# ReubenBond/DistributedRateLimiting.Redis

Hardware: AMD Instinct MI355X
Metric: acquire decisions/sec (node) at 100M keys, 1/2/4/8 GPU; % HBM roofline (higher is better)
Workload: dtype f64; 1 GPU; TokenBucket uniform keys, 2^26-request batches (config B); keys_total=100000000, keys_per_gpu=100000000, batch_per_gpu=67108864, period_ticks=10000000, partitioning=one GPU owns every key

## Files before the change

distributedratelimiting.redis_amd/csrc/tbe_engine.hip:

```cpp
#include <hip/hip_runtime.h>

#include <algorithm>
#include <cmath>
#include <cstdarg>
#include <cstdio>
#include <cstdlib>
#include <cstring>
#include <new>
#include <string>
#include <thread>
#include <tuple>
#include <type_traits>
#include <vector>

#include "../../include/tbe.h"
#include "tbe_device.hpp"
#include "tbe_codec.hpp"
#include "tbe_numfmt.hpp"
#include "tbe_retry.hpp"

#pragma clang fp contract(off)

using namespace tbe;

// ... 96 lines not shown
        const uint32_t k = (uint32_t)v;
        if (k == key) return (nb + (uint32_t)(v >> 32)) << r_bits;
        if (k == kHotEmpty) return key;
        h = (h + 1) & (kHotSlots - 1);
    }
}

template <int N, typename KeyT>
__device__ __forceinline__ void hot_sortkeys(const KeyT (&kv)[N], const uint64_t *slots, uint32_t nb,
                                             int r_bits, uint32_t (&sk)[N]) {
    constexpr int G = N < 4 ? N : 4;
    static_assert(N % G == 0, "groups of G requests");
#pragma unroll
    for (int g = 0; g < N; g += G) {
        uint64_t v1[G], v2[G];
#pragma unroll
        for (int u = 0; u < G; ++u) {
            v1[u] = slots[hot_h1((uint32_t)kv[g + u])];
            v2[u] = slots[hot_h2((uint32_t)kv[g + u])];
        }
#pragma unroll
        for (int u = 0; u < G; ++u) {
            const uint32_t key = (uint32_t)kv[g + u];
            const bool in1 = (uint32_t)v1[u] == key;
            const uint64_t v = in1 ? v1[u] : v2[u];
            sk[g + u] = (in1 || (uint32_t)v2[u] == key) ? (nb + (uint32_t)(v >> 32)) << r_bits : key;
        }
    }
    return;
    uint64_t v[N];
#pragma unroll
    for (int it = 0; it < N; ++it) v[it] = slots[hot_hash((uint32_t)kv[it])];
#pragma unroll
    for (int it = 0; it < N; ++it) {
        const uint32_t key = (uint32_t)kv[it];
        const uint32_t k = (uint32_t)v[it];
        if (k == key) sk[it] = (nb + (uint32_t)(v[it] >> 32)) << r_bits;
        else if (k == kHotEmpty) sk[it] = key;
        else sk[it] = hot_sortkey(key, slots, nb, r_bits);
    }
}

constexpr int kHBlock = 512;
constexpr int kHItems = kTile / kHBlock;
#ifndef TBE_HIST_AHEAD
#define TBE_HIST_AHEAD 1
#endif
#ifndef TBE_HIST_WAVES
#define TBE_HIST_WAVES 8
#endif
#ifndef TBE_HIST_HOT_WAVES
#define TBE_HIST_HOT_WAVES 6
#endif
template <typename KeyT, bool HOT = false>
__global__ __launch_bounds__(kHBlock, HOT ? TBE_HIST_HOT_WAVES : TBE_HIST_WAVES) void k_hist(const KeyT *__restrict__ keys, uint64_t n,
                                                  int shift, uint32_t tiles_per_blk,
                                                  uint32_t ntiles, uint32_t *__restrict__ tileprefix,
                                                  uint32_t *__restrict__ blocksum, uint64_t n_keys,
                                                  uint32_t *__restrict__ err, int validate,
                                                  uint64_t kmask, const HotSet *__restrict__ hot = nullptr,
                                                  uint32_t nb = 0, int r_bits = 0,
                                                  uint32_t *__restrict__ bcount = nullptr,
                                                  int lowbits = 0, uint32_t nbt = 0,
                                                  uint8_t *__restrict__ dig_out = nullptr) {
    __shared__ uint32_t h8[kDigits * 8];
    __shared__ uint32_t tile_lo[2];
    static_assert(kHBlock == 2 * kDigits && kDigits * 8 == 4 * kHBlock, "two threads per digit; 4 counters each");
    __shared__ uint64_t hs[HOT ? kHotLds : 1];
    const int tid = threadIdx.x;
    const bool dig = tid < kDigits;
    const bool any_hot = HOT && hot_load<kHBlock>(hot, hs);
    const uint32_t t0 = blockIdx.x * tiles_per_blk;
    const uint32_t t1 = min(t0 + tiles_per_blk, ntiles);
    uint32_t run = 0;
    uint32_t acc = 0, acc_lo = 0;
    bool bad = false;
    KeyT kn[kHItems];
#if TBE_HIST_AHEAD >= 2
    KeyT kn2[kHItems];
#endif
    auto load_into = [&](KeyT (&dst)[kHItems], uint32_t t) {
#pragma unroll
        for (int it = 0; it < kHItems; ++it) {
            const uint64_t i = (uint64_t)t * kTile + it * kHBlock + tid;
            dst[it] = (t < t1 && i < n) ? LD_P(keys + i) : (KeyT)0;
        }
    };
    load_into(kn, t0);
#if TBE_HIST_AHEAD >= 2
    load_into(kn2, t0 + 1);
#endif
    for (uint32_t t = t0; t < t1; ++t) {
        KeyT kv[kHItems];
#pragma unroll
        for (int it = 0; it < kHItems; ++it) kv[it] = kn[it];
#if TBE_HIST_AHEAD >= 2
#pragma unroll
        for (int it = 0; it < kHItems; ++it) kn[it] = kn2[it];
        load_into(kn2, t + 2);
#else
        load_into(kn, t + 1);
#endif
#pragma unroll
        for (int u = 0; u < 4; ++u) h8[u * kHBlock + tid] = 0;
        __syncthreads();
        const uint64_t base = (uint64_t)t * kTile;
        const uint64_t last = min<uint64_t>(base + kTile, n) - 1;
        uint32_t skv[kHItems];
        if (HOT && any_hot) {
            hot_sortkeys<kHItems>(kv, hot_table(hot, hs), nb, r_bits, skv);
        } else {
#pragma unroll
            for (int it = 0; it < kHItems; ++it) skv[it] = (uint32_t)((uint64_t)kv[it] & kmask);
        }
#pragma unroll
        for (int it = 0; it < kHItems; ++it) {
            const uint64_t i = base + it * kHBlock + tid;
            const bool valid = i < n;
            const uint32_t sk = skv[it];
            const uint32_t d = (sk >> shift) & (kDigits - 1);
            const uint64_t vmask = __ballot(valid);
            const uint32_t d0 = __shfl(d, vmask ? __ffsll((long long)vmask) - 1 : 0, 64);
            if (__all(!valid || d == d0)) {
                if (vmask && (vmask & lanemask_lt()) == 0 && valid) atomicAdd(&h8[d0 * 8], (uint32_t)__popcll(vmask));
            } else {
                if (valid) atomicAdd(&h8[d * 8 + (tid & 7)], 1u);
            }
            if (dig_out && valid) dig_out[i] = (uint8_t)d;
            if (valid) {
                bad |= validate && ((uint64_t)kv[it] >= n_keys);
                if (bcount && (i == base || i == last)) {
                    tile_lo[i == last] = lowbits ? (sk >> r_bits) & ((1u << lowbits) - 1u) : 0u;
                    if (i == base && i == last) tile_lo[0] = tile_lo[1];
                }
            }
        }
        __syncthreads();
        uint32_t c = 0;
        if (dig) {
#pragma unroll
            for (int u = 0; u < 8; ++u) c += h8[tid * 8 + ((u + tid) & 7)];
            tileprefix[(uint64_t)t * kDigits + tid] = run;
            run += c;
        }
        if (bcount) {
            const uint32_t lo0 = tile_lo[0], lo1 = tile_lo[1];
            if (lo0 == lo1) {
                if (dig) {
                    if (lo0 != acc_lo) {
                        const uint32_t bk = ((uint32_t)tid << lowbits) | acc_lo;
                        if (acc && bk < nbt) atomicAdd(&bcount[bk], acc);
                        acc = 0;
                        acc_lo = lo0;
                    }
                    acc += c;
                }
            } else if (lo1 - lo0 < 8) {
                __syncthreads();
#pragma unroll
                for (int u = 0; u < 4; ++u) h8[u * kHBlock + tid] = 0;
                __syncthreads();
#pragma unroll
                for (int it = 0; it < kHItems; ++it) {
                    const uint64_t i = base + it * kHBlock + tid;
                    const uint32_t bk = skv[it] >> r_bits;
                    if (i < n) atomicAdd(&h8[((bk & ((1u << lowbits) - 1u)) - lo0) * kDigits + ((bk >> lowbits) & (kDigits - 1))], 1u);
                }
                __syncthreads();
                if (dig) {
                    for (uint32_t u = 0; u <= lo1 - lo0; ++u) {
                        const uint32_t cnt = h8[u * kDigits + tid];
                        const uint32_t bk = ((uint32_t)tid << lowbits) | (lo0 + u);
                        if (cnt && bk < nbt) atomicAdd(&bcount[bk], cnt);
                    }
                }
            } else {
#pragma unroll
                for (int it = 0; it < kHItems; ++it) {
                    const uint64_t i = base + it * kHBlock + tid;
                    const uint32_t bk = skv[it] >> r_bits;
                    if (i < n && bk < nbt) atomicAdd(&bcount[bk], 1u);
                }
            }
        }
        __syncthreads();
    }
    if (bcount && dig) {
        const uint32_t bk = ((uint32_t)tid << lowbits) | acc_lo;
        if (acc && bk < nbt) atomicAdd(&bcount[bk], acc);
    }
    if (dig) blocksum[(uint64_t)blockIdx.x * kDigits + tid] = run;
    if (__any(bad) && (tid & 63) == 0) atomicOr(err, 1u);
}

__global__ __launch_bounds__(kHBlock, TBE_HIST_WAVES) void k_hist_dig(
    const uint8_t *__restrict__ dig, uint64_t n, uint32_t tiles_per_blk, uint32_t ntiles,
    uint32_t *__restrict__ tileprefix, uint32_t *__restrict__ blocksum,
    const uint32_t *__restrict__ dtot0, uint32_t *__restrict__ bcount, uint32_t nbt) {
    __shared__ uint32_t h8[kDigits * 8];
    __shared__ uint32_t dstart[kDigits + 1];
    __shared__ uint32_t wsum[kHBlock / 64];
    __shared__ uint32_t tlo[kHBlock];
    static_assert(kHBlock == 2 * kDigits && kDigits * 8 == 4 * kHBlock, "two threads per digit; 4 counters each");
    static_assert(kHItems % 8 == 0, "8-byte loads");
    constexpr int kW = kHItems / 8;
    const int tid = threadIdx.x;
    const bool own = tid < kDigits;
    {
        uint32_t all;
        const uint32_t pre = block_excl_scan<kHBlock>(own ? dtot0[tid] : 0u, wsum, &all);
        if (own) dstart[tid] = pre;
        if (tid == 0) dstart[kDigits] = 0xFFFFFFFFu;
    }
    auto d0_of = [&](uint32_t i) {
        uint32_t lo = 0, hi = kDigits;
        while (hi - lo > 1) {
            const uint32_t mid = (lo + hi) >> 1;
            if (dstart[mid] <= i) lo = mid;
            else hi = mid;
        }
        return lo;
    };
    const uint32_t t0 = blockIdx.x * tiles_per_blk;
    const uint32_t t1 = min(t0 + tiles_per_blk, ntiles);
    uint32_t run = 0, acc = 0, acc_lo = 0;
    auto load = [&](uint32_t t, uint64_t (&dst)[kW]) {
#pragma unroll
        for (int q = 0; q < kW; ++q) {
            const uint64_t i = (uint64_t)t * kTile + (uint64_t)tid * kHItems + 8 * q;
            uint64_t v = 0;
            if (t < t1 && i + 8 <= n) {
                v = LD_P(reinterpret_cast<const uint64_t *>(dig + i));
// ... 453 lines not shown
        unpack_rec(rec, ts_orig, tbase0, F, k, p, ts);
        row = k & rmask;
        pos = q;
    }
}

#ifndef TBE_FOLD_FAM
#define TBE_FOLD_FAM 1
#endif
template <int FAM>
__device__ __forceinline__ void fold_input_fam(uint64_t rec, uint32_t q, const FoldFmt &G, int64_t tbase1,
                                               const uint64_t *__restrict__ rec0,
                                               const int64_t *__restrict__ ts_orig, int64_t tbase0,
                                               const PackFmt &F, uint32_t rmask, uint32_t &row, int32_t &p,
                                               int64_t &ts, uint32_t &pos) {
    if (FAM < 0) {
        fold_input(rec, q, G, tbase1, rec0, ts_orig, tbase0, F, rmask, row, p, ts, pos);
    } else if (FAM == 0) {
        uint32_t k;
        unpack_rec(rec, ts_orig, tbase0, F, k, p, ts);
        row = k & rmask;
        pos = q;
    } else {
        row = (uint32_t)(rec & ((1ull << G.rb) - 1));
        p = (int32_t)((rec >> G.rb) & ((1ull << G.pb) - 1));
        pos = (uint32_t)((rec >> (G.rb + G.pb + 1)) & ((1ull << G.pw) - 1));
        if ((rec >> (G.rb + G.pb)) & 1) {
            if (FAM == 1) {
                ts = (int64_t)rec0[pos];
            } else {
                uint32_t k;
                int32_t p0;
                unpack_rec(rec0[pos], ts_orig, tbase0, F, k, p0, ts);
            }
        } else {
            ts = (int64_t)((uint64_t)tbase1 + (rec >> (G.rb + G.pb + 1 + G.pw)));
        }
    }
}

#ifndef TBE_BSCAN_LB
#define TBE_BSCAN_LB 1
#endif
#ifndef TBE_NARROW0
#define TBE_NARROW0 1
#endif
#ifndef TBE_SCATTER0_WAVES
#define TBE_SCATTER0_WAVES 1
#endif
#ifndef TBE_PASS1_CODEC
#define TBE_PASS1_CODEC 1
#endif
constexpr int kLastWaves = 3 * (kPartBlock / 64) / 4;
template <bool FIRST, bool HOT = false, bool IDX = false, bool NOTS = false, bool LAST = false, int FAM = -1>
__global__ __launch_bounds__(kPartBlock, FIRST ? TBE_SCATTER0_WAVES : (FAM >= 0 ? kLastWaves : 1)) void k_scatter_rec(
    const uint64_t *__restrict__ kin, const int32_t *__restrict__ pin, const int64_t *__restrict__ tin,
    const uint64_t *__restrict__ rin, uint64_t n, int shift, PackFmt F,
    const uint32_t *__restrict__ tileprefix, const uint32_t *__restrict__ blockprefix,
    const uint32_t *__restrict__ digit_total, uint32_t tiles_per_blk, uint64_t *__restrict__ rout,
    uint32_t *__restrict__ perm, uint32_t *__restrict__ err, const HotSet *__restrict__ hot = nullptr,
    uint32_t nb = 0, int r_bits = 0, const uint32_t *__restrict__ iin = nullptr,
    uint32_t *__restrict__ iout = nullptr, FoldFmt G = FoldFmt{}, uint8_t *__restrict__ dig_next = nullptr,
    const uint8_t *__restrict__ din = nullptr, int64_t *__restrict__ ts0 = nullptr, Pass1Codec C = Pass1Codec{}) {
    static_assert(!(FIRST && LAST), "fold records come from a pass after the first");
    static_assert(FAM < 0 || LAST, "the record family is fixed only for the last pass");
    const bool n0 = FAM < 0 ? F.n0 != 0 : FAM == 1;
    __shared__ RankLds<kPartBlock> L;
    __shared__ uint32_t goff[kDigits];
    __shared__ uint64_t stage[kTile];
    __shared__ uint16_t stage_e[LAST ? kTile : 1];
    __shared__ uint64_t hs[HOT ? kHotLds : 1];
    static_assert(kPartItems * (kPartBlock / 64) * kDigits * 2 <= kTile * 8, "cnt fits in stage");

    const int tid = threadIdx.x;
    const uint32_t tile = xcd_swizzle(blockIdx.x, gridDim.x);
    const uint64_t base = (uint64_t)tile * kTile;
    const int nv = (int)min((uint32_t)kTile, (uint32_t)(n - base));

    auto body = [&](auto full) {
        constexpr bool FULL = decltype(full)::value;
        const int nvalid = nv;
        uint64_t rec[kPartItems];
        uint32_t key[kPartItems], lpos[kPartItems];
        bool bad = false;
        bool any_hot = false;
        int64_t tv_keep[FIRST ? kPartItems : 1];
        if (FIRST) {
            uint64_t kv[kPartItems];
            int32_t pv[kPartItems];
            int64_t tv[kPartItems];
#pragma unroll
            for (int it = 0; it < kPartItems; ++it) {
                const int e = wb_elem<kPartBlock, kPartItems>(it);
                const bool v = (FULL || e < nvalid);
                kv[it] = v ? LD_P(kin + base + e) : 0ull;
                pv[it] = v ? LD_P(pin + base + e) : 0;
                tv[it] = NOTS ? -1 : (v ? LD_P(tin + base + e) : 0);
            }
            any_hot = HOT && hot_load<kPartBlock>(hot, hs);
            const int64_t tbase = NOTS ? 0 : (n0 ? pack_base32(tin, F) : pack_base(tin, F));
            uint32_t skv[kPartItems];
            if (HOT && any_hot) {
                hot_sortkeys<kPartItems>(kv, hot_table(hot, hs), nb, r_bits, skv);
            } else {
#pragma unroll
                for (int it = 0; it < kPartItems; ++it) skv[it] = (uint32_t)(kv[it] & F.kmask);
            }
#pragma unroll
            for (int it = 0; it < kPartItems; ++it) {
                const int e = wb_elem<kPartBlock, kPartItems>(it);
                bad |= (FULL || e < nvalid) && (pv[it] < 0 || (!NOTS && tv[it] < 0));
                if (n0) {
                    bool esc = false;
                    const uint32_t r32 =
                        NOTS ? (skv[it] & ((1u << F.rb) - 1u)) |
                                   ((uint32_t)(pv[it] < 0 ? 0 : (pv[it] > F.pc_max ? F.pc_max : pv[it])) << F.rb)
                             : pack_rec32(skv[it], pv[it], tv[it], tbase, F, esc);
                    rec[it] = (uint64_t)r32 | ((uint64_t)((skv[it] >> shift) & (kDigits - 1)) << 32) |
                              ((uint64_t)((skv[it] >> (shift + kDigitBits)) & (kDigits - 1)) << 40) |
                              ((uint64_t)esc << 48);
                } else {
                    rec[it] = pack_rec(skv[it], pv[it], tv[it], base + e, tbase, F);
                }
                key[it] = skv[it];
                tv_keep[FIRST ? it : 0] = tv[it];
            }
        } else {
            if (n0) {
                const uint32_t *rin32 = reinterpret_cast<const uint32_t *>(rin);
                uint8_t dv[kPartItems];
#pragma unroll
                for (int it = 0; it < kPartItems; ++it) {
                    const int e = wb_elem<kPartBlock, kPartItems>(it);
                    rec[it] = (FULL || e < nvalid) ? (uint64_t)LD_P(rin32 + base + e) : 0ull;
                    dv[it] = (FULL || e < nvalid) ? din[base + e] : (uint8_t)0;
                }
#pragma unroll
                for (int it = 0; it < kPartItems; ++it) {
                    key[it] = (uint32_t)dv[it] << shift;
                    rec[it] |= (uint64_t)dv[it] << 32;
                }
            } else {
#pragma unroll
                for (int it = 0; it < kPartItems; ++it) {
                    const int e = wb_elem<kPartBlock, kPartItems>(it);
                    rec[it] = (FULL || e < nvalid) ? LD_P(rin + base + e) : 0ull;
                    key[it] = (uint32_t)(rec[it] & F.kmask);
                }
            }
        }
        tile_offsets<kPartBlock>(tile, tiles_per_blk, tileprefix, blockprefix, digit_total, goff, L.wsum);
        rank_tile_wb<kPartBlock, kPartItems, FULL>(key, shift, nvalid, L, reinterpret_cast<uint32_t *>(stage), lpos);
        int64_t tbase0 = 0, tbase1 = 0;
        if (LAST && FAM != 1 && tin) {
            tbase0 = n0 ? pack_base32(tin, F) : pack_base(tin, F);
            tbase1 = fold_base(tin, G);
        }
        __syncthreads();
#pragma unroll
        for (int it = 0; it < kPartItems; ++it) {
            const int e = wb_elem<kPartBlock, kPartItems>(it);
            if (FULL || e < nvalid) {
                const uint32_t d = (key[it] >> shift) & (kDigits - 1);
                stage[lpos[it]] = n0 ? (rec[it] & 0x0000FFFFFFFFFFFFull) : rec[it];
                if (LAST)
                    stage_e[lpos[it]] = (uint16_t)e;
                else if (perm)
                    ST_PERM(perm + base + e, goff[d] + lpos[it] - L.lstart[d]);
                if (FIRST && n0 && ((rec[it] >> 48) & 1u))
                    ts0[goff[d] + lpos[it] - L.lstart[d]] = tv_keep[FIRST ? it : 0];
            }
        }
        __syncthreads();
        uint32_t gpos[kPartItems];
#pragma unroll
        for (int it = 0; it < kPartItems; ++it) {
            const int j = it * kPartBlock + tid;
            if (FULL || j < nvalid) {
                const uint64_t s = stage[j];
                const uint32_t d = n0 ? (uint32_t)(s >> 32) & (kDigits - 1)
                                      : ((uint32_t)(s & F.kmask) >> shift) & (kDigits - 1);
                gpos[it] = goff[d] + (uint32_t)j - L.lstart[d];
                if (n0 && !LAST)
                    reinterpret_cast<uint32_t *>(rout)[gpos[it]] = (uint32_t)s;
                else if (n0)
                    rout[gpos[it]] = FAM == 1 ? fold_rec32_codec((uint32_t)s, (uint32_t)(base + stage_e[j]), C)
                                              : fold_rec32((uint32_t)s, (uint32_t)(base + stage_e[j]), tbase0, tbase1, F, G);
                else
                    rout[gpos[it]] = LAST ? fold_rec(s, (uint32_t)(base + stage_e[j]), tbase0, tbase1, F, G) : s;
                if (!LAST && dig_next)
                    dig_next[gpos[it]] = n0 ? (uint8_t)(s >> 40)
                                            : (uint8_t)(((uint32_t)(s & F.kmask) >> (shift + kDigitBits)) & (kDigits - 1));
            }
        }
        if (IDX) {
            uint32_t *stage32 = reinterpret_cast<uint32_t *>(stage);
            uint32_t iv[kPartItems];
#pragma unroll
            for (int it = 0; it < kPartItems; ++it) {
                const int e = wb_elem<kPartBlock, kPartItems>(it);
                iv[it] = (FULL || e < nvalid) ? (FIRST ? (uint32_t)(base + e) : iin[base + e]) : 0u;
            }
            __syncthreads();
#pragma unroll
            for (int it = 0; it < kPartItems; ++it) {
                const int e = wb_elem<kPartBlock, kPartItems>(it);
                if (FULL || e < nvalid) stage32[lpos[it]] = iv[it];
            }
            __syncthreads();
#pragma unroll
            for (int it = 0; it < kPartItems; ++it) {
                const int j = it * kPartBlock + tid;
                if (FULL || j < nvalid) iout[gpos[it]] = stage32[j];
            }
        }
        if (FIRST && __any(bad) && (tid & 63) == 0) atomicOr(err, 1u);
    };
    if (TBE_FULL_TILE && nv == kTile)
        body(std::true_type{});
// ... 521 lines not shown

constexpr uint32_t kRemNone = 0x3FFFFFFFu;
__device__ __forceinline__ uint32_t pack_wait(uint32_t status, bool evaluated, uint32_t rem) {
    return (status << 30) | (evaluated ? (rem & kRemNone) : kRemNone);
}
constexpr uint32_t kRemNone8 = 63u;
constexpr uint32_t kRemNone16 = 0x3FFFu;
__device__ __forceinline__ void put_wait(uint32_t *res, uint32_t q, uint32_t status, bool evaluated, uint32_t rem,
                                         uint32_t rw) {
    if (rw == 1)
        reinterpret_cast<uint8_t *>(res)[q] = (uint8_t)((status << 6) | (evaluated ? (rem & 63u) : kRemNone8));
    else if (rw == 2)
        reinterpret_cast<uint16_t *>(res)[q] =
            (uint16_t)((status << 14) | (evaluated ? (rem & kRemNone16) : kRemNone16));
    else
        res[q] = pack_wait(status, evaluated, rem);
}
__device__ __forceinline__ uint16_t wait16(uint32_t v) {
    const uint32_t rem = v & kRemNone;
    return (uint16_t)(((v >> 30) << 14) | (rem == kRemNone ? kRemNone16 : (rem & kRemNone16)));
}

template <int W>
__device__ __forceinline__ uint32_t wait_status(uint32_t v) {
    return W == 1 ? v >> 6 : W == 2 ? v >> 14 : v >> 30;
}

template <bool FINAL, bool WAIT, int W = 4, bool RETRY = false>
__global__ __launch_bounds__(kUnBlock) void k_unscatter(uint64_t n, const uint32_t *__restrict__ perm,
                                                          const uint32_t *__restrict__ res_in,
                                                          uint32_t *__restrict__ res_out,
                                                          uint8_t *__restrict__ granted,
                                                          int32_t *__restrict__ remaining,
                                                          const uint32_t *__restrict__ err = nullptr,
                                                          uint32_t *__restrict__ sticky = nullptr,
                                                          const uint32_t *__restrict__ def_in = nullptr,
                                                          uint32_t *__restrict__ def_out = nullptr,
                                                          int64_t *__restrict__ retry = nullptr,
                                                          double rate = 0.0) {
    const int tid = threadIdx.x;
    if (sticky && blockIdx.x == 0 && tid == 0 && *err) *sticky = 1u;
    const uint32_t tile = xcd_swizzle(blockIdx.x, gridDim.x);
    const uint64_t base = (uint64_t)tile * kUnTile;
    const int nvalid = (int)min<uint64_t>(kUnTile, n - base);
    uint32_t pv[kUnItems], r[kUnItems];
#pragma unroll
    for (int it = 0; it < kUnItems; ++it) {
        const int e = it * kUnBlock + tid;
        pv[it] = (e < nvalid) ? LD_U(perm + base + e) : 0u;
    }
#pragma unroll
    for (int it = 0; it < kUnItems; ++it) {
        const int e = it * kUnBlock + tid;
        r[it] = (e < nvalid) ? (W == 1 ? (uint32_t)reinterpret_cast<const uint8_t *>(res_in)[pv[it]]
                                : W == 2 ? (uint32_t)reinterpret_cast<const uint16_t *>(res_in)[pv[it]]
                                         : res_in[pv[it]])
                             : 0u;
    }
    if constexpr (RETRY) {
        uint32_t df[kUnItems];
#pragma unroll
        for (int it = 0; it < kUnItems; ++it) {
            const int e = it * kUnBlock + tid;
            df[it] = (e < nvalid && wait_status<W>(r[it]) == TBE_WAIT_FAILED) ? def_in[pv[it]] : 0u;
        }
#pragma unroll
        for (int it = 0; it < kUnItems; ++it) {
            const int e = it * kUnBlock + tid;
            if (e >= nvalid) continue;
            const bool failed = wait_status<W>(r[it]) == TBE_WAIT_FAILED;
            if (FINAL) ST_U(retry + base + e, failed ? retry_ticks(df[it], rate) : (int64_t)TBE_RETRY_NONE);
            else if (failed) def_out[base + e] = df[it];
        }
    }
#pragma unroll
    for (int it = 0; it < kUnItems; ++it) {
        const int e = it * kUnBlock + tid;
        if (e >= nvalid) continue;
        const uint64_t i = base + e;
        if (FINAL && WAIT && W == 1) {
            ST_U(granted + i, (uint8_t)(r[it] >> 6));
            const uint32_t rem = r[it] & 63u;
            ST_U(remaining + i, (rem == kRemNone8) ? -1 : (int32_t)rem);
        } else if (FINAL && WAIT && W == 2) {
            ST_U(granted + i, (uint8_t)(r[it] >> 14));
            const uint32_t rem = r[it] & kRemNone16;
            ST_U(remaining + i, (rem == kRemNone16) ? -1 : (int32_t)rem);
        } else if (FINAL && WAIT) {
            ST_U(granted + i, (uint8_t)(r[it] >> 30));
            const uint32_t rem = r[it] & kRemNone;
            ST_U(remaining + i, (rem == kRemNone) ? -1 : (int32_t)rem);
        } else if (FINAL && W == 1) {
            ST_U(granted + i, (uint8_t)(r[it] >> 7));
            ST_U(remaining + i, (int32_t)(r[it] & 0x7Fu));
        } else if (FINAL) {
            ST_U(granted + i, (uint8_t)(r[it] >> 31));
            ST_U(remaining + i, (int32_t)(r[it] & 0x7FFFFFFFu));
        } else if (W == 1) {
            ST_U(reinterpret_cast<uint8_t *>(res_out) + i, (uint8_t)r[it]);
        } else if (W == 2) {
            ST_U(reinterpret_cast<uint16_t *>(res_out) + i, (uint16_t)r[it]);
        } else {
            ST_U(res_out + i, r[it]);
        }
    }
}
// ... 16 lines not shown
    const uint64_t base = (uint64_t)tile * kTile;
    const int nvalid = (int)min<uint64_t>(kTile, n - base);
    uint32_t dg[kPartItems], lpos[kPartItems];
#pragma unroll
    for (int it = 0; it < kPartItems; ++it) {
        const int e = wb_elem<kPartBlock, kPartItems>(it);
        dg[it] = e < nvalid ? (uint32_t)LD_U(digit + base + e) : 0u;
    }
    tile_offsets<kPartBlock>(tile, tiles_per_blk, tileprefix, blockprefix, digit_total, goff, L.wsum);
    rank_tile_wb<kPartBlock, kPartItems>(dg, 0, nvalid, L, wcnt, lpos);
    uint32_t r[kPartItems];
#pragma unroll
    for (int it = 0; it < kPartItems; ++it) {
        const int e = wb_elem<kPartBlock, kPartItems>(it);
        const uint32_t q = goff[dg[it]] + lpos[it] - L.lstart[dg[it]];
        r[it] = e < nvalid ? (W == 1   ? (uint32_t)reinterpret_cast<const uint8_t *>(res_in)[q]
                              : W == 2 ? (uint32_t)reinterpret_cast<const uint16_t *>(res_in)[q]
                                       : res_in[q])
                           : 0u;
    }
    if constexpr (RETRY) {
#pragma unroll
        for (int it = 0; it < kPartItems; ++it) {
            const int e = wb_elem<kPartBlock, kPartItems>(it);
            if (e >= nvalid) continue;
            const uint32_t q = goff[dg[it]] + lpos[it] - L.lstart[dg[it]];
            const bool failed = wait_status<W>(r[it]) == TBE_WAIT_FAILED;
            ST_U(retry + base + e, failed ? retry_ticks(def_in[q], rate) : (int64_t)TBE_RETRY_NONE);
        }
    }
#pragma unroll
    for (int it = 0; it < kPartItems; ++it) {
        const int e = wb_elem<kPartBlock, kPartItems>(it);
        if (e >= nvalid) continue;
        const uint64_t i = base + e;
        if (WAIT && W == 1) {
            ST_U(granted + i, (uint8_t)(r[it] >> 6));
            const uint32_t rem = r[it] & 63u;
            ST_U(remaining + i, (rem == kRemNone8) ? -1 : (int32_t)rem);
        } else if (WAIT && W == 2) {
            ST_U(granted + i, (uint8_t)(r[it] >> 14));
            const uint32_t rem = r[it] & kRemNone16;
            ST_U(remaining + i, (rem == kRemNone16) ? -1 : (int32_t)rem);
        } else if (WAIT) {
            ST_U(granted + i, (uint8_t)(r[it] >> 30));
            const uint32_t rem = r[it] & kRemNone;
            ST_U(remaining + i, (rem == kRemNone) ? -1 : (int32_t)rem);
        } else if (W == 1) {
            ST_U(granted + i, (uint8_t)(r[it] >> 7));
            ST_U(remaining + i, (int32_t)(r[it] & 0x7Fu));
        } else {
            ST_U(granted + i, (uint8_t)(r[it] >> 31));
            ST_U(remaining + i, (int32_t)(r[it] & 0x7FFFFFFFu));
        }
    }
}

constexpr int kSegBlock = kFoldBlock;
constexpr int kSegItems = 16;
constexpr uint32_t kSeg = kSegBlock * kSegItems;

struct SegSummary {
    int64_t max_ts;
    int32_t min_p;
    uint32_t pad;
};
struct SegState {
    Slot s;
    double ft;
    uint32_t pass;
    uint32_t pad;
};


__device__ __forceinline__ uint32_t seg_run(const uint32_t *segbase, uint32_t j) {
    uint32_t lo = 0, hi = kHotKeysMax;
    while (hi - lo > 1) {
        const uint32_t mid = (lo + hi) >> 1;
        if (segbase[mid] <= j) lo = mid;
        else hi = mid;
    }
    return lo;
}

template <bool SPEC>
__global__ __launch_bounds__(kSegBlock) void k_hot_summary(
    const uint64_t *__restrict__ srec, const int64_t *__restrict__ ts_orig, PackFmt F,
    const uint32_t *__restrict__ bstart, uint32_t nb, uint32_t *segbase,
    SegSummary *__restrict__ summ, const uint32_t *__restrict__ err, FoldFmt G, const uint64_t *__restrict__ rec0,
    const HotSet *__restrict__ hot = nullptr, const Slot *__restrict__ table = nullptr, TbParams P = TbParams{},
    uint32_t *__restrict__ res = nullptr, uint32_t narrow = 0, uint32_t plan = 0) {
    __shared__ int64_t wts[kSegBlock / 64];
    __shared__ int32_t wp[kSegBlock / 64];
    __shared__ uint32_t pass_s0;
    __shared__ uint32_t sb[kHotKeysMax + 1];
    __shared__ uint32_t sbw[kSegBlock / 64];
    if (*err) return;
    const int tid = threadIdx.x, lane = tid & 63, w = tid >> 6;
    if (plan) {
        static_assert(kHotKeysMax == 2 * kSegBlock, "two runs per thread");
        const uint32_t cnt = hot->count;
        uint32_t ns[2];
#pragma unroll
        for (int u = 0; u < 2; ++u) {
            const uint32_t h = 2 * tid + u;
            ns[u] = h < cnt ? (bstart[nb + h + 1] - bstart[nb + h] + kSeg - 1) / kSeg : 0u;
// ... 2013 lines not shown
    }
    return G;
}

tbe_status run_batch(tbe_engine *e, const uint64_t *keys, const int32_t *permits,
                     const int64_t *ts, uint64_t n, uint8_t *granted, int32_t *remaining,
                     hipStream_t caller, int64_t id_base = 0, hipEvent_t in_ready = nullptr,
                     hipStream_t out_stream = nullptr, uint32_t ai_base = 0, int64_t *retry = nullptr) {
    const bool approx = e->cfg.kind == TBE_KIND_APPROXIMATE;
    const bool wait = e->cfg.kind != TBE_KIND_TOKEN_BUCKET;
    if (n == 0) return TBE_OK;
    if (n >= (1ull << 32)) return fail(e, TBE_EINVAL, "batch of %llu requests exceeds 2^32-1",
                                       (unsigned long long)n);
    if (e->packed && !approx && !ts) return fail(e, TBE_EINVAL, "null timestamps");
    const bool pipe = e->pipeline;
    Workspace &w = e->ws[pipe ? e->ws_cur : 0];
    tbe_status rc = ensure_workspace(e, w, n);
    if (rc != TBE_OK) return rc;
    if (retry) {
        if (!w.def[0]) HIP_TRY(e, hipMalloc(&w.def[0], w.cap_n * sizeof(uint32_t)));
        if (!w.def[1] && e->passes - (batch_fold_fmt(e, n).on ? 2 : 1) >= 1)
            HIP_TRY(e, hipMalloc(&w.def[1], w.cap_n * sizeof(uint32_t)));
    }
    uint32_t ntiles, nblk, tpb;
    tiles_for(n, ntiles, nblk, tpb);
    hipStream_t sf = caller ? caller : e->stream, sp = sf;
    if (pipe) {
        sf = e->stream;
        sp = e->pstream;
        if (in_ready) {
            HIP_TRY(e, hipStreamWaitEvent(sp, in_ready, 0));
        } else if (caller) {
            HIP_TRY(e, hipEventRecord(e->ev_in, caller));
            HIP_TRY(e, hipStreamWaitEvent(sp, e->ev_in, 0));
        }
        if (w.used) HIP_TRY(e, hipStreamWaitEvent(sp, w.done, 0));
        if (w.hot_pending) HIP_TRY(e, hipStreamWaitEvent(sp, w.hot_done, 0));
    } else if (in_ready) {
        HIP_TRY(e, hipStreamWaitEvent(sf, in_ready, 0));
    }
    HIP_TRY(e, hipMemsetAsync(w.bcount, 0, ((uint64_t)e->nb_total + 2) * sizeof(uint32_t), sp));
    if (w.bs_fresh) {
        HIP_TRY(e, hipMemsetAsync(w.bsflags, 0, kBsMaxBlocks * sizeof(unsigned long long), sp));
        w.bs_fresh = false;
    }

    const uint64_t kmask = e->packed ? e->pf.kmask : ~0ull;
    const FoldFmt G = batch_fold_fmt(e, n);
    PackFmt pf = e->pf;
    pf.n0 = G.n0;
    const uint64_t *rec0 = G.on ? (G.n0 ? reinterpret_cast<const uint64_t *>(w.ts0) : w.pass[e->passes - 2].rec)
                                : nullptr;
    const bool unrank = e->unrank;
    const unsigned fold_grid = G.on ? (unsigned)((1ull << G.region_bits) * G.n_hi) : e->nbuckets;
    const uint32_t tb_wmin = (!approx && !wait) ? fold_wide_min(e, n) : 1u;
    const bool sparse_tb = tb_wmin > 1u;
    const bool hot_on = e->hot_cap && !(sparse_tb && n < (1ull << TBE_HOT_SPARSE_MIN_LOG2));
    HotSet *hot = hot_on ? e->hot[e->nbatch % 3] : nullptr;
    HotSet *hot_next = hot_on ? e->hot[(e->nbatch + 2) % 3] : nullptr;
    if (hot && n >= kHotSampleMin) k_hot_sample<<<1, 1024, 0, sp>>>(keys, n, e->cfg.n_keys, hot, e->hot_cap);
    for (int p = 0; p < e->passes; ++p) {
        const int shift = e->r_bits + kDigitBits * p;
        PassBufs &out = w.pass[p];
        stage_begin(e, ST_HIST, sp);
        uint32_t *bc = (p == e->passes - 1) ? w.bcount : nullptr;
        const int lowbits = kDigitBits * p;
        uint8_t *dig = (p == 0 && unrank) ? w.dig0 : nullptr;
        uint8_t *dnext = (p == 0 && e->dig1) ? w.dig1 : nullptr;
        if (p == 0 && hot)
            k_hist<uint64_t, true><<<nblk, kHBlock, 0, sp>>>(keys, n, shift, tpb, ntiles, out.tileprefix,
                                                             w.blocksum, e->cfg.n_keys, w.err, 1, kmask,
                                                             hot, e->nbuckets, e->r_bits, bc, lowbits,
                                                             e->nb_total, dig);
        else if (p == 0)
            k_hist<uint64_t><<<nblk, kHBlock, 0, sp>>>(keys, n, shift, tpb, ntiles, out.tileprefix,
                                                       w.blocksum, e->cfg.n_keys, w.err, 1, kmask,
                                                       nullptr, e->nbuckets, e->r_bits, bc, lowbits,
                                                       e->nb_total, dig);
        else if (e->dig1 && p == 1)
            k_hist_dig<<<nblk, kHBlock, 0, sp>>>(w.dig1, n, tpb, ntiles, out.tileprefix, w.blocksum,
                                                 w.pass[0].digit_total, bc, e->nb_total);
        else if (e->packed)
            k_hist<uint64_t><<<nblk, kHBlock, 0, sp>>>(w.pass[p - 1].rec, n, shift, tpb, ntiles,
                                                       out.tileprefix, w.blocksum, e->cfg.n_keys,
                                                       w.err, 0, kmask, nullptr, e->nbuckets,
                                                       e->r_bits, bc, lowbits, e->nb_total);
        else
            k_hist<uint32_t><<<nblk, kHBlock, 0, sp>>>(w.pass[p - 1].keys, n, shift, tpb, ntiles,
                                                       out.tileprefix, w.blocksum, e->cfg.n_keys,
                                                       w.err, 0, kmask, nullptr, e->nbuckets,
                                                       e->r_bits, bc, lowbits, e->nb_total);
        stage_end(e, ST_HIST, sp);
        stage_begin(e, ST_COLSCAN, sp);
        k_colscan<<<kDigits, kBlock, 0, sp>>>(w.blocksum, nblk, out.blockprefix, out.digit_total);
        stage_end(e, ST_COLSCAN, sp);
        stage_begin(e, ST_SCATTER, sp);
#define LAUNCH_LAST_FAM(IDXK, FAMK, iin_, iout_)                                                               \
    k_scatter_rec<false, false, IDXK, false, true, FAMK><<<ntiles, kPartBlock, 0, sp>>>(                       \
        nullptr, nullptr, ts, w.pass[p - 1].rec, n, shift, pf, out.tileprefix, out.blockprefix,                \
        out.digit_total, tpb, out.rec, nullptr, w.err, nullptr, 0, 0, iin_, iout_, G, nullptr, w.dig1, nullptr, \
        pass1_codec(pf, G, true))
#define LAUNCH_LAST(IDXK, iin_, iout_)                                                     \
    do {                                                                                   \
        if (TBE_PASS1_CODEC && G.n0 && pass1_codec_ok(pf, G))                              \
            LAUNCH_LAST_FAM(IDXK, 1, iin_, iout_);                                         \
        else if (TBE_PASS1_CODEC && !G.n0)                                                 \
            LAUNCH_LAST_FAM(IDXK, 0, iin_, iout_);                                         \
        else                                                                               \
            LAUNCH_LAST_FAM(IDXK, -1, iin_, iout_);                                        \
    } while (0)
        if (e->packed && approx && p == 0)
            k_scatter_rec<true, false, false, true><<<ntiles, kPartBlock, 0, sp>>>(
                keys, permits, nullptr, nullptr, n, shift, pf, out.tileprefix, out.blockprefix,
                out.digit_total, tpb, out.rec, unrank ? nullptr : out.perm, w.err, nullptr, 0, 0, nullptr,
                nullptr, FoldFmt{}, dnext);
        else if (e->packed && approx && G.on && p == e->passes - 1)
            k_scatter_rec<false, false, false, false, true><<<ntiles, kPartBlock, 0, sp>>>(
                nullptr, nullptr, nullptr, w.pass[p - 1].rec, n, shift, pf, out.tileprefix,
                out.blockprefix, out.digit_total, tpb, out.rec, nullptr, w.err, nullptr, 0, 0, nullptr,
                nullptr, G, nullptr, w.dig1);
        else if (e->packed && approx)
            k_scatter_rec<false><<<ntiles, kPartBlock, 0, sp>>>(
                nullptr, nullptr, nullptr, w.pass[p - 1].rec, n, shift, e->pf, out.tileprefix,
                out.blockprefix, out.digit_total, tpb, out.rec, out.perm, w.err);
        else if (e->packed && wait && p == 0)
            k_scatter_rec<true, false, true><<<ntiles, kPartBlock, 0, sp>>>(
                keys, permits, ts, nullptr, n, shift, pf, out.tileprefix, out.blockprefix,
                out.digit_total, tpb, out.rec, unrank ? nullptr : out.perm, w.err, nullptr, 0, 0, nullptr, out.idx,
                FoldFmt{}, dnext, nullptr, w.ts0);
        else if (e->packed && wait && G.on && p == e->passes - 1)
            LAUNCH_LAST_FAM(true, -1, w.pass[p - 1].idx, out.idx);
        else if (e->packed && wait)
            k_scatter_rec<false, false, true><<<ntiles, kPartBlock, 0, sp>>>(
                nullptr, nullptr, nullptr, w.pass[p - 1].rec, n, shift, e->pf, out.tileprefix,
                out.blockprefix, out.digit_total, tpb, out.rec, out.perm, w.err, nullptr, 0, 0,
                w.pass[p - 1].idx, out.idx);
        else if (e->packed && p == 0 && hot)
            k_scatter_rec<true, true><<<ntiles, kPartBlock, 0, sp>>>(
                keys, permits, ts, nullptr, n, shift, pf, out.tileprefix, out.blockprefix,
                out.digit_total, tpb, out.rec, unrank ? nullptr : out.perm, w.err, hot, e->nbuckets, e->r_bits,
                nullptr, nullptr, FoldFmt{}, dnext, nullptr, w.ts0);
        else if (e->packed && p == 0)
            k_scatter_rec<true><<<ntiles, kPartBlock, 0, sp>>>(
                keys, permits, ts, nullptr, n, shift, pf, out.tileprefix, out.blockprefix,
                out.digit_total, tpb, out.rec, unrank ? nullptr : out.perm, w.err, nullptr, 0, 0, nullptr,
                nullptr, FoldFmt{}, dnext, nullptr, w.ts0);
        else if (e->packed && G.on && p == e->passes - 1)
            LAUNCH_LAST(false, nullptr, nullptr);
        else if (e->packed)
            k_scatter_rec<false><<<ntiles, kPartBlock, 0, sp>>>(
                nullptr, nullptr, nullptr, w.pass[p - 1].rec, n, shift, e->pf, out.tileprefix,
                out.blockprefix, out.digit_total, tpb, out.rec, out.perm, w.err);
        else if (approx && p == 0)
            k_scatter<uint64_t, true, false><<<ntiles, kPartBlock, 0, sp>>>(
                keys, permits, nullptr, nullptr, n, shift, out.tileprefix, out.blockprefix,
                out.digit_total, tpb, out.keys, out.permits, nullptr, out.idx, out.perm, w.err, 1);
        else if (approx)
            k_scatter<uint32_t, true, false><<<ntiles, kPartBlock, 0, sp>>>(
                w.pass[p - 1].keys, w.pass[p - 1].permits, nullptr, w.pass[p - 1].idx, n, shift,
                out.tileprefix, out.blockprefix, out.digit_total, tpb, out.keys, out.permits, nullptr,
                out.idx, out.perm, w.err, 0);
        else if (p == 0 && !wait)
            k_scatter<uint64_t, false><<<ntiles, kPartBlock, 0, sp>>>(
                keys, permits, ts, nullptr, n, shift, out.tileprefix, out.blockprefix,
                out.digit_total, tpb, out.keys, out.permits, out.ts, nullptr, out.perm, w.err, 1);
        else if (p == 0)
            k_scatter<uint64_t, true><<<ntiles, kPartBlock, 0, sp>>>(
                keys, permits, ts, nullptr, n, shift, out.tileprefix, out.blockprefix,
                out.digit_total, tpb, out.keys, out.permits, out.ts, out.idx, out.perm, w.err, 1);
        else if (!wait)
            k_scatter<uint32_t, false><<<ntiles, kPartBlock, 0, sp>>>(
                w.pass[p - 1].keys, w.pass[p - 1].permits, w.pass[p - 1].ts, nullptr, n, shift,
                out.tileprefix, out.blockprefix, out.digit_total, tpb, out.keys, out.permits,
                out.ts, nullptr, out.perm, w.err, 0);
        else
            k_scatter<uint32_t, true><<<ntiles, kPartBlock, 0, sp>>>(
                w.pass[p - 1].keys, w.pass[p - 1].permits, w.pass[p - 1].ts, w.pass[p - 1].idx,
                n, shift, out.tileprefix, out.blockprefix, out.digit_total, tpb, out.keys,
                out.permits, out.ts, out.idx, out.perm, w.err, 0);
        stage_end(e, ST_SCATTER, sp);
    }
    const PassBufs &sorted = w.pass[e->passes - 1];
    stage_begin(e, ST_BOUNDS, sp);
    const uint32_t bs_blocks = (e->nb_total + kBsTile - 1) / kBsTile;
    if (TBE_BSCAN_LB && bs_blocks <= kBsMaxBlocks) {
        if (++w.bs_tag == 0) {
            HIP_TRY(e, hipMemsetAsync(w.bsflags, 0, kBsMaxBlocks * sizeof(unsigned long long), sp));
            w.bs_tag = 1;
        }
// ... 113 lines not shown
        if (pipe) {
            HIP_TRY(e, hipEventRecord(e->ev_hot, sf));
            HIP_TRY(e, hipStreamWaitEvent(e->hstream, e->ev_hot, 0));
            k_hot_update<<<1, 1024, 0, e->hstream>>>(hot_next, e->hot_cap - hot_reserve_host(e->hot_cap), w.err);
            HIP_TRY(e, hipEventRecord(w.hot_done, e->hstream));
            w.hot_pending = true;
        } else {
            k_hot_update<<<1, 1024, 0, sf>>>(hot_next, e->hot_cap - hot_reserve_host(e->hot_cap), w.err);
        }
        stage_end(e, ST_HOT, sf);
    }
    stage_begin(e, ST_UNSCATTER, sf);
    const unsigned untiles = (unsigned)((n + kUnTile - 1) / kUnTile);
    int cur = 0;
    for (int p = e->passes - (G.on ? 2 : 1); p >= 1; --p) {
        if (retry && e->medium)
            k_unscatter<false, false, 2, true><<<untiles, kUnBlock, 0, sf>>>(
                n, w.pass[p].perm, w.res[cur], w.res[cur ^ 1], nullptr, nullptr, nullptr, nullptr, w.def[cur],
                w.def[cur ^ 1]);
        else if (retry)
            k_unscatter<false, false, 4, true><<<untiles, kUnBlock, 0, sf>>>(
                n, w.pass[p].perm, w.res[cur], w.res[cur ^ 1], nullptr, nullptr, nullptr, nullptr, w.def[cur],
                w.def[cur ^ 1]);
        else if (e->narrow && !approx)
            k_unscatter<false, false, 1><<<untiles, kUnBlock, 0, sf>>>(n, w.pass[p].perm, w.res[cur],
                                                                   w.res[cur ^ 1], nullptr, nullptr);
        else if (e->medium)
            k_unscatter<false, false, 2><<<untiles, kUnBlock, 0, sf>>>(n, w.pass[p].perm, w.res[cur],
                                                                   w.res[cur ^ 1], nullptr, nullptr);
        else
            k_unscatter<false, false><<<untiles, kUnBlock, 0, sf>>>(n, w.pass[p].perm, w.res[cur],
                                                                    w.res[cur ^ 1], nullptr, nullptr);
        cur ^= 1;
    }
#define TBE_UNRANK(...)                                                                             \
    __VA_ARGS__<<<ntiles, kPartBlock, 0, sf>>>(n, w.dig0, w.pass[0].tileprefix, w.pass[0].blockprefix, \
                                               w.pass[0].digit_total, tpb, w.res[cur], granted, remaining)
    if (retry && unrank && e->medium)
        k_unrank<2, true, true><<<ntiles, kPartBlock, 0, sf>>>(
            n, w.dig0, w.pass[0].tileprefix, w.pass[0].blockprefix, w.pass[0].digit_total, tpb, w.res[cur],
            granted, remaining, w.def[cur], retry, e->ap.decay_rate);
    else if (retry && unrank)
        k_unrank<4, true, true><<<ntiles, kPartBlock, 0, sf>>>(
            n, w.dig0, w.pass[0].tileprefix, w.pass[0].blockprefix, w.pass[0].digit_total, tpb, w.res[cur],
            granted, remaining, w.def[cur], retry, e->ap.decay_rate);
    else if (retry && e->medium)
        k_unscatter<true, true, 2, true><<<untiles, kUnBlock, 0, sf>>>(
            n, w.pass[0].perm, w.res[cur], nullptr, granted, remaining, w.err, e->sticky, w.def[cur], nullptr,
            retry, e->ap.decay_rate);
    else if (retry)
        k_unscatter<true, true, 4, true><<<untiles, kUnBlock, 0, sf>>>(
            n, w.pass[0].perm, w.res[cur], nullptr, granted, remaining, w.err, e->sticky, w.def[cur], nullptr,
            retry, e->ap.decay_rate);
    else if (unrank && !wait && e->narrow)
        TBE_UNRANK(k_unrank<1>);
    else if (unrank && !wait)
        TBE_UNRANK(k_unrank<4>);
    else if (unrank && e->narrow)
        TBE_UNRANK(k_unrank<1, true>);
    else if (unrank && e->medium)
        TBE_UNRANK(k_unrank<2, true>);
    else if (unrank)
        TBE_UNRANK(k_unrank<4, true>);
#undef TBE_UNRANK
    else if (e->narrow && !wait && !approx)
        k_unscatter<true, false, 1><<<untiles, kUnBlock, 0, sf>>>(n, w.pass[0].perm, w.res[cur],
                                                                  nullptr, granted, remaining,
            w.err, e->sticky);
    else if (wait && e->narrow)
        k_unscatter<true, true, 1><<<untiles, kUnBlock, 0, sf>>>(n, w.pass[0].perm, w.res[cur],
                                                                 nullptr, granted, remaining,
            w.err, e->sticky);
    else if (wait && e->medium)
        k_unscatter<true, true, 2><<<untiles, kUnBlock, 0, sf>>>(n, w.pass[0].perm, w.res[cur],
                                                                 nullptr, granted, remaining,
            w.err, e->sticky);
    else if (wait)
        k_unscatter<true, true><<<untiles, kUnBlock, 0, sf>>>(n, w.pass[0].perm, w.res[cur],
                                                              nullptr, granted, remaining,
            w.err, e->sticky);
    else
        k_unscatter<true, false><<<untiles, kUnBlock, 0, sf>>>(n, w.pass[0].perm, w.res[cur],
                                                               nullptr, granted, remaining,
            w.err, e->sticky);
    stage_end(e, ST_UNSCATTER, sf);
    if (unrank) k_sticky<<<1, 64, 0, sf>>>(w.err, e->sticky);
    HIP_TRY(e, hipGetLastError());
    if (pipe) {
        HIP_TRY(e, hipEventRecord(w.done, sf));
        w.used = true;
        hipStream_t outs = out_stream ? out_stream : caller;
        if (outs && outs != sf) {
            HIP_TRY(e, hipEventRecord(e->ev_out, sf));
            HIP_TRY(e, hipStreamWaitEvent(outs, e->ev_out, 0));
        }
        e->ws_cur ^= 1;
    } else if (out_stream && out_stream != sf) {
        HIP_TRY(e, hipEventRecord(e->ev_out, sf));
        HIP_TRY(e, hipStreamWaitEvent(out_stream, e->ev_out, 0));
    }
    e->last_err = w.err;
    ++e->nbatch;
    return TBE_OK;
}

}
// ... 1634 lines not shown
```

Measured before the change: 43.20 billion decisions/s.

## Store tile-local 16-bit permutation and unpartition replies via per-digit coalesced runs

```diff
diff --git a/distributedratelimiting.redis_amd/csrc/tbe_engine.hip b/distributedratelimiting.redis_amd/csrc/tbe_engine.hip
--- a/distributedratelimiting.redis_amd/csrc/tbe_engine.hip
+++ b/distributedratelimiting.redis_amd/csrc/tbe_engine.hip
@@ -172,6 +172,10 @@
 #ifndef TBE_HIST_HOT_WAVES
 #define TBE_HIST_HOT_WAVES 6
 #endif
+#ifndef TBE_HIST_LOAD16
+#define TBE_HIST_LOAD16 0
+#endif
+typedef uint64_t u64x2 __attribute__((ext_vector_type(2)));
 template <typename KeyT, bool HOT = false>
 __global__ __launch_bounds__(kHBlock, HOT ? TBE_HIST_HOT_WAVES : TBE_HIST_WAVES) void k_hist(const KeyT *__restrict__ keys, uint64_t n,
                                                   int shift, uint32_t tiles_per_blk,
@@ -199,7 +203,25 @@
 #if TBE_HIST_AHEAD >= 2
     KeyT kn2[kHItems];
 #endif
+    constexpr bool kLoad16 = TBE_HIST_LOAD16 && sizeof(KeyT) == 8;
+    const bool al16 = kLoad16 && (reinterpret_cast<uintptr_t>(keys) & 15u) == 0;
+    auto wide = [&](uint32_t t) { return al16 && t < t1 && ((uint64_t)t + 1) * kTile <= n; };
+    auto elem = [&](bool w16, int it) {
+        return w16 ? (uint32_t)((((it >> 1) * kHBlock + tid) << 1) | (it & 1)) : (uint32_t)(it * kHBlock + tid);
+    };
     auto load_into = [&](KeyT (&dst)[kHItems], uint32_t t) {
+        if constexpr (kLoad16) {
+            if (wide(t)) {
+                const u64x2 *k2 = reinterpret_cast<const u64x2 *>(keys + (uint64_t)t * kTile);
+#pragma unroll
+                for (int s = 0; s < kHItems / 2; ++s) {
+                    const u64x2 v = LD_P(k2 + s * kHBlock + tid);
+                    dst[2 * s] = (KeyT)v.x;
+                    dst[2 * s + 1] = (KeyT)v.y;
+                }
+                return;
+            }
+        }
 #pragma unroll
         for (int it = 0; it < kHItems; ++it) {
             const uint64_t i = (uint64_t)t * kTile + it * kHBlock + tid;
@@ -225,6 +247,7 @@
         for (int u = 0; u < 4; ++u) h8[u * kHBlock + tid] = 0;
         __syncthreads();
         const uint64_t base = (uint64_t)t * kTile;
+        const bool w16 = wide(t);
         const uint64_t last = min<uint64_t>(base + kTile, n) - 1;
         uint32_t skv[kHItems];
         if (HOT && any_hot) {
@@ -235,7 +258,7 @@
         }
 #pragma unroll
         for (int it = 0; it < kHItems; ++it) {
-            const uint64_t i = base + it * kHBlock + tid;
+            const uint64_t i = base + elem(w16, it);
             const bool valid = i < n;
             const uint32_t sk = skv[it];
             const uint32_t d = (sk >> shift) & (kDigits - 1);
@@ -282,7 +305,7 @@
                 __syncthreads();
 #pragma unroll
                 for (int it = 0; it < kHItems; ++it) {
-                    const uint64_t i = base + it * kHBlock + tid;
+                    const uint64_t i = base + elem(w16, it);
                     const uint32_t bk = skv[it] >> r_bits;
                     if (i < n) atomicAdd(&h8[((bk & ((1u << lowbits) - 1u)) - lo0) * kDigits + ((bk >> lowbits) & (kDigits - 1))], 1u);
                 }
@@ -297,7 +320,7 @@
             } else {
 #pragma unroll
                 for (int it = 0; it < kHItems; ++it) {
-                    const uint64_t i = base + it * kHBlock + tid;
+                    const uint64_t i = base + elem(w16, it);
                     const uint32_t bk = skv[it] >> r_bits;
                     if (i < n && bk < nbt) atomicAdd(&bcount[bk], 1u);
                 }
@@ -857,7 +880,7 @@
 #define TBE_PASS1_CODEC 1
 #endif
 constexpr int kLastWaves = 3 * (kPartBlock / 64) / 4;
-template <bool FIRST, bool HOT = false, bool IDX = false, bool NOTS = false, bool LAST = false, int FAM = -1>
+template <bool FIRST, bool HOT = false, bool IDX = false, bool NOTS = false, bool LAST = false, int FAM = -1, bool P16 = false>
 __global__ __launch_bounds__(kPartBlock, FIRST ? TBE_SCATTER0_WAVES : (FAM >= 0 ? kLastWaves : 1)) void k_scatter_rec(
     const uint64_t *__restrict__ kin, const int32_t *__restrict__ pin, const int64_t *__restrict__ tin,
     const uint64_t *__restrict__ rin, uint64_t n, int shift, PackFmt F,
@@ -869,6 +892,7 @@
     const uint8_t *__restrict__ din = nullptr, int64_t *__restrict__ ts0 = nullptr, Pass1Codec C = Pass1Codec{}) {
     static_assert(!(FIRST && LAST), "fold records come from a pass after the first");
     static_assert(FAM < 0 || LAST, "the record family is fixed only for the last pass");
+    static_assert(!P16 || FIRST, "tile-local permutation entries are pass 0's");
     const bool n0 = FAM < 0 ? F.n0 != 0 : FAM == 1;
     __shared__ RankLds<kPartBlock> L;
     __shared__ uint32_t goff[kDigits];
@@ -970,6 +994,8 @@
                 stage[lpos[it]] = n0 ? (rec[it] & 0x0000FFFFFFFFFFFFull) : rec[it];
                 if (LAST)
                     stage_e[lpos[it]] = (uint16_t)e;
+                else if (P16)
+                    ST_PERM(reinterpret_cast<uint16_t *>(perm) + base + e, (uint16_t)lpos[it]);
                 else if (perm)
                     ST_PERM(perm + base + e, goff[d] + lpos[it] - L.lstart[d]);
                 if (FIRST && n0 && ((rec[it] >> 48) & 1u))
@@ -1597,6 +1623,12 @@
 #pragma unroll
     for (int it = 0; it < kUnItems; ++it) {
         const int e = it * kUnBlock + tid;
+#ifdef TBE_UN_NO_GATHER
+        if (FINAL) {
+            asm volatile("" ::"v"(pv[it]));
+            pv[it] = (uint32_t)(base + e);
+        }
+#endif
         r[it] = (e < nvalid) ? (W == 1 ? (uint32_t)reinterpret_cast<const uint8_t *>(res_in)[pv[it]]
                                 : W == 2 ? (uint32_t)reinterpret_cast<const uint16_t *>(res_in)[pv[it]]
                                          : res_in[pv[it]])
@@ -1719,6 +1751,132 @@
         } else {
             ST_U(granted + i, (uint8_t)(r[it] >> 31));
             ST_U(remaining + i, (int32_t)(r[it] & 0x7FFFFFFFu));
+        }
+    }
+}
+
+#ifndef TBE_UNPART_RUNS
+#define TBE_UNPART_RUNS 1
+#endif
+constexpr int kRunTasks1 = 3 * kPartBlock;
+static_assert(kTile / 4 + 3 * kDigits / 2 <= kRunTasks1, "every run: its dwords, plus at most 1.5 for its ragged ends");
+template <int W>
+__global__ __launch_bounds__(kPartBlock, 8) void k_unpart_runs(
+    uint64_t n, const uint16_t *__restrict__ idx, const uint32_t *__restrict__ tileprefix,
+    const uint32_t *__restrict__ blockprefix, const uint32_t *__restrict__ digit_total,
+    uint32_t tiles_per_blk, uint32_t ntiles, uint32_t nblk, const uint32_t *__restrict__ res_in,
+    uint8_t *__restrict__ granted, int32_t *__restrict__ remaining, const uint32_t *__restrict__ err,
+    uint32_t *__restrict__ sticky) {
+    static_assert(W == 1 || W == 4, "one-byte or four-byte replies");
+    static_assert(kTile == 8 * kPartBlock && kPartBlock >= kDigits && kPartItems == 8, "8 indices (16 bytes) per thread");
+    using R = std::conditional_t<W == 1, uint8_t, uint32_t>;
+    constexpr int kTasks = W == 1 ? kRunTasks1 : kTile;
+    constexpr int kPer = kTasks / kPartBlock;
+    __shared__ uint32_t goff[kDigits];
+    __shared__ uint32_t lst[kDigits];
+    __shared__ uint32_t rcnt[kDigits];
+    __shared__ uint32_t tst[kDigits];
+    __shared__ uint32_t wsum[kPartBlock / 64];
+    __shared__ uint32_t wmax[kPartBlock / 64];
+    __shared__ __attribute__((aligned(16))) uint8_t tdig[kTile];
+    __shared__ __attribute__((aligned(16))) uint16_t lidx[kTile];
+    __shared__ R reply[kTile];
+    const int tid = threadIdx.x, lane = tid & 63, w = tid >> 6;
+    if (sticky && blockIdx.x == 0 && tid == 0 && *err) *sticky = 1u;
+    const uint32_t tile = xcd_swizzle(blockIdx.x, gridDim.x);
+    const uint64_t base = (uint64_t)tile * kTile;
+    const int nvalid = (int)min<uint64_t>(kTile, n - base);
+    const u32x4 iv = LD_U(reinterpret_cast<const u32x4 *>(idx + base) + tid);
+    uint32_t cnt = 0;
+    if (tid < kDigits) {
+        const uint32_t blk = tile / tiles_per_blk;
+        const uint32_t tp = tileprefix[(uint64_t)tile * kDigits + tid];
+        if (tile + 1 < ntiles && (tile + 1) % tiles_per_blk != 0) {
+            cnt = tileprefix[(uint64_t)(tile + 1) * kDigits + tid] - tp;
+        } else {
+            const uint32_t bp = blockprefix[(uint64_t)blk * kDigits + tid];
+            const uint32_t nx = blk + 1 < nblk ? blockprefix[(uint64_t)(blk + 1) * kDigits + tid] : digit_total[tid];
+            cnt = nx - bp - tp;
+        }
+    }
+    tile_offsets<kPartBlock>(tile, tiles_per_blk, tileprefix, blockprefix, digit_total, goff, wsum);
+    const uint32_t g = tid < kDigits ? goff[tid] : 0u;
+    const uint32_t ntask = W == 1 ? (cnt ? ((g & 3u) + cnt + 3u) >> 2 : 0u) : cnt;
+    uint32_t all;
+    const uint32_t sc = block_excl_scan<kPartBlock>(cnt | (ntask << 16), wsum, &all);
+    const uint32_t lstart = sc & 0xFFFFu, tstart = sc >> 16;
+    const uint32_t ntasks = all >> 16;
+    reinterpret_cast<uint2 *>(tdig)[tid] = make_uint2(0u, 0u);
+    reinterpret_cast<u32x4 *>(lidx)[tid] = iv;
+    __syncthreads();
+    if (tid < kDigits) {
+        lst[tid] = lstart;
+        rcnt[tid] = cnt;
+        tst[tid] = tstart;
+        if (cnt) tdig[tstart] = (uint8_t)tid;
+    }
+    __syncthreads();
+    {
+        const uint2 v = reinterpret_cast<const uint2 *>(tdig)[tid];
+        uint32_t b[8];
+#pragma unroll
+        for (int k = 0; k < 8; ++k) b[k] = ((k < 4 ? v.x : v.y) >> (8 * (k & 3))) & 0xFFu;
+#pragma unroll
+        for (int k = 1; k < 8; ++k) b[k] = max(b[k], b[k - 1]);
+        uint32_t inc = b[7];
+#pragma unroll
+        for (int o = 1; o < 64; o <<= 1) {
+            const uint32_t y = __shfl_up(inc, o, 64);
+            if (lane >= o) inc = max(inc, y);
+        }
+        uint32_t carry = __shfl_up(inc, 1, 64);
+        if (lane == 0) carry = 0;
+        if (lane == 63) wmax[w] = inc;
+        __syncthreads();
+#pragma unroll
+        for (int j = 0; j < kPartBlock / 64; ++j) carry = max(carry, j < w ? wmax[j] : 0u);
+        uint2 o2 = make_uint2(0u, 0u);
+#pragma unroll
+        for (int k = 0; k < 8; ++k) {
+            const uint32_t d = max(b[k], carry);
+            if (k < 4) o2.x |= d << (8 * k);
+            else o2.y |= d << (8 * (k - 4));
+        }
+        reinterpret_cast<uint2 *>(tdig)[tid] = o2;
+    }
+    __syncthreads();
+#pragma unroll
+    for (int it = 0; it < kPer; ++it) {
+        const uint32_t k = (uint32_t)(it * kPartBlock + tid);
+        if (k >= ntasks) continue;
+        const uint32_t d = tdig[k];
+        const uint32_t gd = goff[d], t = k - tst[d];
+        if constexpr (W == 1) {
+            const uint32_t a = (gd & ~3u) + 4u * t;
+            const uint32_t v = res_in[a >> 2];
+            const uint32_t c = rcnt[d], s = lst[d];
+#pragma unroll
+            for (uint32_t bb = 0; bb < 4; ++bb) {
+                const uint32_t p = a + bb - gd;
+                if (p < c) reply[s + p] = (uint8_t)(v >> (8 * bb));
+            }
+        } else {
+            reply[k] = res_in[gd + t];
+        }
+    }
+    __syncthreads();
+#pragma unroll
+    for (int it = 0; it < kPartItems; ++it) {
+        const int e = it * kPartBlock + tid;
+        if (e >= nvalid) continue;
+        const uint64_t i = base + e;
+        const uint32_t r = reply[lidx[e] & (kTile - 1)];
+        if (W == 1) {
+            ST_U(granted + i, (uint8_t)(r >> 7));
+            ST_U(remaining + i, (int32_t)(r & 0x7Fu));
+        } else {
+            ST_U(granted + i, (uint8_t)(r >> 31));
+            ST_U(remaining + i, (int32_t)(r & 0x7FFFFFFFu));
         }
     }
 }
@@ -3838,6 +3996,7 @@
     const uint64_t *rec0 = G.on ? (G.n0 ? reinterpret_cast<const uint64_t *>(w.ts0) : w.pass[e->passes - 2].rec)
                                 : nullptr;
     const bool unrank = e->unrank;
+    const bool runs = TBE_UNPART_RUNS && e->packed && !approx && !wait && !unrank && !retry;
     const unsigned fold_grid = G.on ? (unsigned)((1ull << G.region_bits) * G.n_hi) : e->nbuckets;
     const uint32_t tb_wmin = (!approx && !wait) ? fold_wide_min(e, n) : 1u;
     const bool sparse_tb = tb_wmin > 1u;
@@ -3921,6 +4080,16 @@
                 nullptr, nullptr, nullptr, w.pass[p - 1].rec, n, shift, e->pf, out.tileprefix,
                 out.blockprefix, out.digit_total, tpb, out.rec, out.perm, w.err, nullptr, 0, 0,
                 w.pass[p - 1].idx, out.idx);
+        else if (e->packed && p == 0 && hot && runs)
+            k_scatter_rec<true, true, false, false, false, -1, true><<<ntiles, kPartBlock, 0, sp>>>(
+                keys, permits, ts, nullptr, n, shift, pf, out.tileprefix, out.blockprefix,
+                out.digit_total, tpb, out.rec, out.perm, w.err, hot, e->nbuckets, e->r_bits,
+                nullptr, nullptr, FoldFmt{}, dnext, nullptr, w.ts0);
+        else if (e->packed && p == 0 && runs)
+            k_scatter_rec<true, false, false, false, false, -1, true><<<ntiles, kPartBlock, 0, sp>>>(
+                keys, permits, ts, nullptr, n, shift, pf, out.tileprefix, out.blockprefix,
+                out.digit_total, tpb, out.rec, out.perm, w.err, nullptr, 0, 0, nullptr,
+                nullptr, FoldFmt{}, dnext, nullptr, w.ts0);
         else if (e->packed && p == 0 && hot)
             k_scatter_rec<true, true><<<ntiles, kPartBlock, 0, sp>>>(
                 keys, permits, ts, nullptr, n, shift, pf, out.tileprefix, out.blockprefix,
@@ -4140,6 +4309,14 @@
         k_unscatter<true, true, 4, true><<<untiles, kUnBlock, 0, sf>>>(
             n, w.pass[0].perm, w.res[cur], nullptr, granted, remaining, w.err, e->sticky, w.def[cur], nullptr,
             retry, e->ap.decay_rate);
+    else if (runs && e->narrow)
+        k_unpart_runs<1><<<ntiles, kPartBlock, 0, sf>>>(
+            n, reinterpret_cast<const uint16_t *>(w.pass[0].perm), w.pass[0].tileprefix, w.pass[0].blockprefix,
+            w.pass[0].digit_total, tpb, ntiles, nblk, w.res[cur], granted, remaining, w.err, e->sticky);
+    else if (runs)
+        k_unpart_runs<4><<<ntiles, kPartBlock, 0, sf>>>(
+            n, reinterpret_cast<const uint16_t *>(w.pass[0].perm), w.pass[0].tileprefix, w.pass[0].blockprefix,
+            w.pass[0].digit_total, tpb, ntiles, nblk, w.res[cur], granted, remaining, w.err, e->sticky);
     else if (unrank && !wait && e->narrow)
         TBE_UNRANK(k_unrank<1>);
     else if (unrank && !wait)
```

Result: faster. 44.67 billion decisions/s, median of 6 (+3.4%).
